# PaddlePaddle/PASSL

Measured on AMD Instinct MI355X. Metric: images/sec/node (2-view), MoCo-v2 R50 bs256/GPU, higher is better.
Workload: dtype bf16; 1 GPU; MoCo-v2 ResNet-50 bf16, bs=256/GPU, 2x224^2 synthetic views, queue=65536, dim=128, T=0.2, m=0.999, momentum-SGD (BASELINE configs[1]); global_batch=256, parallelism=dp1, allocator_retries=0

## Files before the change

include/passl_hip.h:

```cpp
#ifndef PASSL_HIP_H_
#define PASSL_HIP_H_

#include <stdint.h>

#ifdef __cplusplus
extern "C" {
#endif

typedef void* passl_stream_t;

enum passl_status {
  PASSL_OK = 0,
  PASSL_EINVAL = -1,
  PASSL_ELAUNCH = -2,
  PASSL_EUNSUPPORTED = -3
};

enum passl_dtype { PASSL_F32 = 0, PASSL_BF16 = 1 };

#define PASSL_HIP_ABI_VERSION 16
int passl_hip_abi_version(void);
int passl_hip_set_option(const char* name, int value);
int passl_hip_get_option(const char* name, int* value);
int passl_hip_last_igemm_kernel(void);
// ... 147 lines not shown
                           int C, int relu, int dtype, passl_stream_t stream);

int passl_hip_maxpool3x3s2_fwd(const void* x, void* y, uint8_t* idx, int N, int H, int W, int C,
                               int dtype, passl_stream_t stream);
int passl_hip_maxpool3x3s2_bwd(const void* dy, const uint8_t* idx, void* dx, int N, int H, int W,
                               int C, int dtype, passl_stream_t stream);
int passl_hip_bn_relu_maxpool_blocks(int N, int H, int W, int C);
int passl_hip_bn_relu_maxpool_fwd(const void* x, const float* scale, const float* shift, void* y, uint8_t* idx, int N,
                                  int H, int W, int C, int dtype, passl_stream_t stream);
int passl_hip_bn_relu_maxpool_bwd_reduce(const void* dy, const uint8_t* idx, const void* x, const float* mean,
                                         const float* invstd, const float* scale, const float* shift, float* partial,
                                         int nblocks, int N, int H, int W, int C, int dtype, passl_stream_t stream);
int passl_hip_bn_relu_maxpool_bwd_apply(const void* dy, const uint8_t* idx, const void* x, const float* coef,
                                        const float* scale, const float* shift, void* dx, int N, int H, int W, int C,
                                        int dtype, passl_stream_t stream);
int passl_hip_avgpool_fwd(const void* x, void* y, int N, int HW, int C, int dtype,
                          passl_stream_t stream);
int passl_hip_avgpool_bwd(const void* dy, void* dx, int N, int HW, int C, int dtype,
                          passl_stream_t stream);
int passl_hip_relu_bwd(const void* dy, const void* y, void* dx, int64_t n, int dtype,
                       passl_stream_t stream);
int passl_hip_colsum(const void* x, float* out, int64_t M, int C, int dtype, float* ws,
                     int64_t ws_floats, passl_stream_t stream);
int passl_hip_colsum_acc(const void* x, float* out, int64_t M, int C, int dtype, float* ws,
                         int64_t ws_floats, passl_stream_t stream);


int passl_hip_l2norm_fwd(const float* x, float* y, float* norm, int N, int D, float eps,
                         passl_stream_t stream);
int passl_hip_l2norm_bwd(const float* dy, const float* y, const float* norm, void* dx, int N,
// ... 197 lines not shown
```

passl_amd/csrc/bn_chunk.h:

```cpp
#pragma once
#include "common.h"

namespace bnc {

__device__ __forceinline__ void affine8(float (&v)[8], const float (&sc)[8], const float (&sh)[8]) {
#pragma unroll
  for (int e = 0; e < 8; ++e) v[e] = v[e] * sc[e] + sh[e];
}

__device__ __forceinline__ void relu8(float (&v)[8]) {
#pragma unroll
  for (int e = 0; e < 8; ++e) v[e] = fmaxf(v[e], 0.f);
}

__device__ __forceinline__ void bwd8(float (&o)[8], const float (&g)[8], const float (&v)[8], const float (&cA)[8],
                                     const float (&cB)[8], const float (&cC)[8]) {
#pragma unroll
  for (int e = 0; e < 8; ++e) o[e] = __fmaf_rn(cA[e], g[e], cB[e] * v[e]) + cC[e];
}

}
```

passl_amd/csrc/stem_pool.hip:

```cpp
#include "common.h"
#include "options.h"

namespace {

constexpr int kThreads = 256;
constexpr int kUnroll = 8;

template <typename T> __device__ __forceinline__ float round_to(float v);
template <> __device__ __forceinline__ float round_to<float>(float v) { return v; }
template <> __device__ __forceinline__ float round_to<bf16_t>(float v) { return bf2f(f2bf(v)); }

template <typename T>
__global__ void __launch_bounds__(kThreads) bn_relu_maxpool_fwd_kernel(const T* __restrict__ x,
                                                                       const float* __restrict__ scale,
                                                                       const float* __restrict__ shift,
                                                                       T* __restrict__ y, uint8_t* __restrict__ idx,
                                                                       int N, int H, int W, int C, int P, int Q) {
  const uint32_t cc = (uint32_t)C >> 3;
  const uint32_t total = (uint32_t)N * P * Q * cc;
  const uint32_t i = blockIdx.x * kThreads + threadIdx.x;
  if (i >= total) return;
  const int c8 = (int)(i % cc);
  uint32_t t = i / cc;
  const int q = (int)(t % (uint32_t)Q); t /= (uint32_t)Q;
// ... 236 lines not shown
template <typename T>
struct Item {
  uint32_t gw[2][2][kWords<T>];
  uint32_t ix[2][2][2];
  uint32_t xv[2][2][kWords<T>];
  uint32_t xb;
  uint32_t flags;
};

template <typename T>
__device__ __forceinline__ const T* at(const T* base, uint32_t elem_off) {
  return reinterpret_cast<const T*>(reinterpret_cast<const char*>(base) + (size_t)(elem_off * (uint32_t)sizeof(T)));
}

template <typename T>
__device__ __forceinline__ void load_item(Item<T>& it, const T* __restrict__ dy, const uint8_t* __restrict__ idx,
                                          const T* __restrict__ x, const Geo& g, uint32_t i, int c8) {
  const bool live = i < g.total;
  const uint32_t pix = (live ? i : g.total - 1) >> g.cshift;
  const uint32_t t1 = fdiv(pix, g.dW2);
  const uint32_t q2 = pix - t1 * g.W2;
  const uint32_t n = fdiv(t1, g.dH2);
  const uint32_t p2 = t1 - n * g.H2;
  const uint32_t C = (uint32_t)g.C;
  const bool pv = p2 + 1 < (uint32_t)g.P, qv = q2 + 1 < (uint32_t)g.Q;
  const bool hv = 2 * p2 + 1 < (uint32_t)g.H, wv = 2 * q2 + 1 < (uint32_t)g.W;
  const uint32_t ob = ((n * (uint32_t)g.P + p2) * (uint32_t)g.Q + q2) * C + (uint32_t)c8 * 8u;
  const uint32_t oa = pv ? (uint32_t)g.Q * C : 0u, oq = qv ? C : 0u;
  const uint32_t xb = ((n * (uint32_t)g.H + 2 * p2) * (uint32_t)g.W + 2 * q2) * C + (uint32_t)c8 * 8u;
  const uint32_t xa = hv ? (uint32_t)g.W * C : 0u, xq = wv ? C : 0u;
#pragma unroll
  for (int a = 0; a < 2; ++a)
#pragma unroll
    for (int b = 0; b < 2; ++b) {
      const uint32_t o = ob + (a ? oa : 0u) + (b ? oq : 0u);
      load_raw<T>(at<T>(dy, o), it.gw[a][b]);
      const uint2 t = *reinterpret_cast<const uint2*>(idx + (size_t)o);
      it.ix[a][b][0] = t.x; it.ix[a][b][1] = t.y;
    }
#pragma unroll
  for (int dh = 0; dh < 2; ++dh)
#pragma unroll
    for (int dw = 0; dw < 2; ++dw) load_raw<T>(at<T>(x, xb + (dh ? xa : 0u) + (dw ? xq : 0u)), it.xv[dh][dw]);
  it.xb = xb;
  const uint32_t l = live ? 1u : 0u, p1 = pv ? l : 0u, q1 = qv ? l : 0u, h1 = hv ? l : 0u, w1 = wv ? l : 0u;
  it.flags = l | (q1 << 1) | (p1 << 2) | ((p1 & q1) << 3) | (l << 4) | (w1 << 5) | (h1 << 6) | ((h1 & w1) << 7);
}

template <typename T>
__device__ __forceinline__ void pair_grad(const Item<T>& it, const uint32_t (&ix)[2][2][2], int k, const float (&sc)[2],
                                          const float (&sh)[2], float (&g)[2][2][2], float (&xf)[2][2][2]) {
  float w[2][2][2];
  uint32_t t[2][2][2];
#pragma unroll
  for (int a = 0; a < 2; ++a)
#pragma unroll
    for (int b = 0; b < 2; ++b)
#pragma unroll
      for (int j = 0; j < 2; ++j) {
        w[a][b][j] = elem<T>(it.gw[a][b], 2 * k + j);
        t[a][b][j] = __builtin_amdgcn_ubfe(ix[a][b][k >> 1], (uint32_t)(16 * (k & 1) + 8 * j), 8u);
// ... 104 lines not shown
#pragma unroll
  for (int e = 0; e < 8; ++e) { red[threadIdx.x * 16 + e] = a0[e]; red[threadIdx.x * 16 + 8 + e] = a1[e]; }
  __syncthreads();
  const uint32_t cc = 1u << g.cshift;
  if (threadIdx.x < cc) {
    float s0[8] = {0, 0, 0, 0, 0, 0, 0, 0}, s1[8] = {0, 0, 0, 0, 0, 0, 0, 0};
    for (uint32_t l = 0; l < kThreads / cc; ++l) {
      const uint32_t t = l * cc + threadIdx.x;
#pragma unroll
      for (int e = 0; e < 8; ++e) { s0[e] += red[t * 16 + e]; s1[e] += red[t * 16 + 8 + e]; }
    }
    float* o = partial + ((int64_t)blockIdx.x * g.C + threadIdx.x * 8) * 2;
#pragma unroll
    for (int e = 0; e < 8; e += 2) *reinterpret_cast<float4*>(o + e * 2) = make_float4(s0[e], s1[e], s0[e + 1], s1[e + 1]);
  }
}

}

bool shape_ok(int N, int H, int W, int C, int64_t* out_items, int64_t* in_items) {
  if (N <= 0 || H <= 0 || W <= 0 || C <= 0 || (C & 7) || (kThreads % (C >> 3)) != 0) return false;
  const int P = (H + 2 - 3) / 2 + 1, Q = (W + 2 - 3) / 2 + 1;
  *out_items = (int64_t)N * P * Q * (C >> 3);
  *in_items = (int64_t)N * ((H + 1) / 2) * ((W + 1) / 2) * (C >> 3);
  return *out_items <= 0x7fffffffll && *in_items <= 0x7fffffffll && (int64_t)N * H * W * C <= 0x7fffffff0ll;
}

v2::Geo make_geo(int N, int H, int W, int C, int64_t in_items) {
  v2::Geo g;
  g.H = H; g.W = W; g.C = C;
// ... 72 lines not shown
                                                   const float* scale, const float* shift, void* dx, int N, int H, int W,
                                                   int C, int dtype, passl_stream_t stream) {
  int64_t oi, ii;
  if (!dy || !idx || !x || !coef || !scale || !shift || !dx || !aligned16(dy) || !aligned16(x) || !aligned16(dx) ||
      !aligned16(coef) || !aligned16(scale) || !aligned16(shift) || (reinterpret_cast<uintptr_t>(idx) & 7))
    return PASSL_EINVAL;
  if (!shape_ok(N, H, W, C, &oi, &ii)) return PASSL_EUNSUPPORTED;
  const int P = (H + 2 - 3) / 2 + 1, Q = (W + 2 - 3) / 2 + 1;
  PASSL_DISPATCH_DTYPE(dtype, hipLaunchKernelGGL(bn_relu_maxpool_bwd_apply_kernel<T>, dim3((unsigned)((ii + kThreads - 1) / kThreads)),
                                                 dim3(kThreads), 0, as_stream(stream), reinterpret_cast<const T*>(dy), idx,
                                                 reinterpret_cast<const T*>(x), coef, scale, shift, reinterpret_cast<T*>(dx), N,
                                                 H, W, C, P, Q);)
  PASSL_RETURN_IF_LAUNCH_FAILED();
  return PASSL_OK;
}
```

passl_amd/hip/config.py:

```python
import os

import torch

_state = {'device': None, 'dtype': torch.bfloat16,
          'fused_bn_stats': os.environ.get('PASSL_FUSED_BN_STATS', '1') != '0',
          'fuse_residual_grad': os.environ.get('PASSL_FUSE_RESIDUAL_GRAD', '1') != '0',
          'fused_bn_backward': os.environ.get('PASSL_FUSED_BN_BACKWARD', '1') != '0',
          'fused_bn_backward2': os.environ.get('PASSL_FUSED_BN_BACKWARD2', '1') != '0',
          'overlap': os.environ.get('PASSL_OVERLAP', '1') != '0',
          'fork_downsample': os.environ.get('PASSL_FORK_DOWNSAMPLE', '1') != '0',
          'side_reductions': os.environ.get('PASSL_SIDE_REDUCTIONS', '1') != '0',
          'fused_stem_pool': os.environ.get('PASSL_FUSED_STEM_POOL', '1') != '0',
          'stem_wgrad_parts': max(1, int(os.environ.get('PASSL_STEM_WGRAD_PARTS', '2') or 1)),
          'stem_tail_flush': os.environ.get('PASSL_STEM_TAIL_FLUSH', '1') != '0',
          'stem_wgrad_main_last': os.environ.get('PASSL_STEM_WGRAD_MAIN_LAST', '1') != '0',
          'side_urgent_rows': int(os.environ.get('PASSL_SIDE_URGENT_ROWS', '500000') or 0),
          'wgrad_halo': int(os.environ.get('PASSL_WGRAD_HALO', '2') or 0),
          'igemm_a_bn': int(os.environ.get('PASSL_IGEMM_A_BN', '0') or 0) & 7,
          'igemm_a_bnb': int(os.environ.get('PASSL_IGEMM_A_BNB', '7') or 0) & 7}


def set_device(name):
    if isinstance(name, torch.device):
        _state['device'] = name
    elif name in ('gpu', 'cuda'):
        _state['device'] = torch.device('cuda', int(os.environ.get('PASSL_DEVICE_INDEX',
                                                                  os.environ.get('LOCAL_RANK', 0))))
        torch.cuda.set_device(_state['device'])
# ... 59 lines not shown
    return _state['fork_downsample']


def side_reductions():
    return _state['side_reductions']


def fused_stem_pool():
    return _state['fused_stem_pool']


def stem_wgrad_parts():
    return _state['stem_wgrad_parts']


def stem_wgrad_main_last():
    return _state['stem_wgrad_main_last']


def side_urgent_rows():
    return _state['side_urgent_rows']


def stem_tail_flush():
    return _state['stem_tail_flush']


def wgrad_halo():
    return _state['wgrad_halo']


def igemm_a_bn(channels):
    return bool(_state['igemm_a_bn'] & _ktile_bit(channels))


def igemm_a_bnb(channels):
    return bool(_state['igemm_a_bnb'] & _ktile_bit(channels))


def _ktile_bit(channels):
    nk = (channels + 63) // 64
    return 1 if nk == 1 else (2 if nk == 2 else 4)


_BOOL_FLAGS = ('fused_bn_stats', 'fuse_residual_grad', 'fused_bn_backward', 'overlap', 'fork_downsample',
               'side_reductions', 'fused_stem_pool', 'fused_bn_backward2', 'stem_tail_flush', 'stem_wgrad_main_last')
_INT_FLAGS = ('stem_wgrad_parts', 'side_urgent_rows', 'wgrad_halo', 'igemm_a_bn', 'igemm_a_bnb')


def set_flag(name, value):
    if name in _BOOL_FLAGS:
        _state[name] = bool(value)
    elif name in _INT_FLAGS:
        _state[name] = max(1, int(value)) if name == 'stem_wgrad_parts' else int(value)
        if name == 'wgrad_halo':
            from . import lib as L
            if L.loaded():
                L.check(L.load().passl_hip_set_option(b'wgrad_halo', int(value)), 'set_option wgrad_halo')
    else:
        raise KeyError('unknown flag %r (known: %s)' % (name, ', '.join(_BOOL_FLAGS + _INT_FLAGS)))

# ... 5 lines not shown
```

passl_amd/hip/lib.py:

```python
import ctypes as C
import os

import torch

_HERE = os.path.dirname(os.path.abspath(__file__))
LIB_PATH = os.path.join(os.path.dirname(_HERE), 'lib', 'libpassl_hip.so')

F32, BF16 = 0, 1
ABI_VERSION = 16
GRAD_CLIP_CHUNK = 16384
_DT = {torch.float32: F32, torch.bfloat16: BF16}

c_p = C.c_void_p
c_i = C.c_int
c_l = C.c_int64
c_f = C.c_float


class ConvDesc(C.Structure):
    _fields_ = [('a', c_p), ('b', c_p), ('y', c_p), ('scale', c_p), ('shift', c_p),
                ('residual', c_p), ('stats', c_p),
                ('bnb_y', c_p), ('bnb_mask', c_p), ('bnb_mean', c_p), ('bnb_invstd', c_p),
                ('bnb_scale', c_p), ('bnb_shift', c_p), ('bnb_partial', c_p),
                ('N', C.c_int32), ('OP', C.c_int32), ('OQ', C.c_int32), ('NCOLS', C.c_int32),
# ... 57 lines not shown
                                      c_i, c_p]),
    'passl_hip_bn_bwd_finalize': (c_i, [c_p, c_i, c_l, c_i, c_p, c_p, c_p, c_p, c_p, c_p, c_p]),
    'passl_hip_bn_moments': (c_i, [c_p, c_i, c_l, c_i, c_i, c_p, c_p]),
    'passl_hip_bn_finalize_moments': (c_i, [c_p, c_i, c_i, c_p, c_p, c_p, c_p, c_f, c_f, c_p, c_p, c_p, c_p, c_p]),
    'passl_hip_bn_bwd_sums': (c_i, [c_p, c_i, c_l, c_i, c_p, c_p]),
    'passl_hip_bn_bwd_finalize_sums': (c_i, [c_p, c_i, c_i, c_l, c_i, c_p, c_p, c_p, c_p, c_p, c_p, c_p]),
    'passl_hip_bn_bwd_apply': (c_i, [c_p, c_p, c_p, c_p, c_p, c_p, c_p, c_p, c_l, c_i, c_i, c_i,
                                     c_p]),
    'passl_hip_maxpool3x3s2_fwd': (c_i, [c_p, c_p, c_p, c_i, c_i, c_i, c_i, c_i, c_p]),
    'passl_hip_maxpool3x3s2_bwd': (c_i, [c_p, c_p, c_p, c_i, c_i, c_i, c_i, c_i, c_p]),
    'passl_hip_bn_relu_maxpool_blocks': (c_i, [c_i, c_i, c_i, c_i]),
    'passl_hip_bn_relu_maxpool_fwd': (c_i, [c_p, c_p, c_p, c_p, c_p, c_i, c_i, c_i, c_i, c_i, c_p]),
    'passl_hip_bn_relu_maxpool_bwd_reduce': (c_i, [c_p, c_p, c_p, c_p, c_p, c_p, c_p, c_p, c_i, c_i, c_i, c_i, c_i, c_i,
                                                   c_p]),
    'passl_hip_bn_relu_maxpool_bwd_apply': (c_i, [c_p, c_p, c_p, c_p, c_p, c_p, c_p, c_i, c_i, c_i, c_i, c_i, c_p]),
    'passl_hip_avgpool_fwd': (c_i, [c_p, c_p, c_i, c_i, c_i, c_i, c_p]),
    'passl_hip_avgpool_bwd': (c_i, [c_p, c_p, c_i, c_i, c_i, c_i, c_p]),
    'passl_hip_relu_bwd': (c_i, [c_p, c_p, c_p, c_l, c_i, c_p]),
    'passl_hip_colsum': (c_i, [c_p, c_p, c_l, c_i, c_i, c_p, c_l, c_p]),
    'passl_hip_colsum_acc': (c_i, [c_p, c_p, c_l, c_i, c_i, c_p, c_l, c_p]),
    'passl_hip_l2norm_fwd': (c_i, [c_p, c_p, c_p, c_i, c_i, c_f, c_p]),
    'passl_hip_l2norm_bwd': (c_i, [c_p, c_p, c_p, c_p, c_i, c_i, c_i, c_p]),
    'passl_hip_infonce_workspace_bytes': (c_l, [c_i, c_i]),
    'passl_hip_infonce_fwd': (c_i, [c_p, c_p, c_p, c_i, c_i, c_i, c_f, c_p, c_p, c_p, c_p, c_p]),
    'passl_hip_infonce_bwd_workspace_bytes': (c_l, [c_i, c_i]),
    'passl_hip_infonce_bwd': (c_i, [c_p, c_p, c_p, c_p, c_p, c_i, c_i, c_i, c_f, c_p, c_p, c_p]),
    'passl_hip_enqueue': (c_i, [c_p, c_p, c_i, c_i, c_i, c_i, c_p]),
    'passl_hip_enqueue_dev': (c_i, [c_p, c_p, c_i, c_i, c_p, c_i, c_p]),
    'passl_hip_lars_momentum': (c_i, [c_p, c_p, c_p, c_p, c_p, c_p, c_i, c_p, c_i, c_p, c_f, c_f,
                                      c_f, c_f, c_f, c_p]),
# ... 174 lines not shown
```

passl_amd/hip/nn.py:

```python
from types import SimpleNamespace

import torch
import torch.nn as tnn
from torch.autograd import Function

from . import config, ops, streams
from . import plan as P
from .packer import WeightPacker


class Layer(tnn.Module):

    def sublayers(self, include_self=False):
        mods = list(self.modules())
        return mods if include_self else mods[1:]

    def set_state_dict(self, sd, *a, **k):
        return self.load_state_dict(sd, *a, **k)


def _need_rt(layer):
    if getattr(layer, '_rt', None) is None:
        raise RuntimeError('%s is not attached to an EncoderArena (call EncoderArena(encoder) after '
                           'building the model)' % type(layer).__name__)
# ... 75 lines not shown


def dy_link(t):
    return getattr(t, '_passl_dy_link', None)


def _apply_in_consumer(conv, y, residual, relu, stats):
    g = conv.geom
    return (relu and residual is None and stats is not None and y.dtype == torch.bfloat16 and not conv.is_stem and
            g.k == 1 and g.stride == 1 and g.pad == 0 and g.cin == y.shape[-1] and g.cin % 64 == 0 and g.cin < 512 and
            g.cout > 64 and config.igemm_a_bn(g.cin))


class WgradLink:

    __slots__ = ('launch', 'done')

    def __init__(self):
        self.launch = None
        self.done = False


def wgrad_link(t):
    return getattr(t, '_passl_wgrad_link', None)


def _stem_wgrad(layer, pl, x, dy, tmp):
    ops.conv_wgrad(pl.wd, x, dy.reshape(-1, layer.geom.cout), tmp)


def _stem_wgrad_finish(layer, tmp):
    ops.unpad_add(tmp, layer._rt.dw, layer.geom.cout, 7, 7, 3, P.STEM_ROW // 4, 4)


# ... 10 lines not shown
        if pending is not None:
            done = ops.conv_igemm(pl.fd, pending.y, rt.w_fwd, y, stats=slab,
                                  apro=dict(mode=1, scale=pending.scale, shift=pending.shift, out=x))
            if done is None:
                ops.bn_apply(pending.y, pending.scale, pending.shift, None, True, out=x)
        if done is None:
            ops.conv_igemm(pl.fd, x, rt.w_fwd, y, stats=slab)
        if any(ctx.needs_input_grad):
            rt.arena.expect_grad(rt.indices)
        ctx.save_for_backward(x)
        ctx.layer, ctx.pl, ctx.hw = layer, pl, hw
        ctx.add_slot, ctx.sink_slot, ctx.producer = add_slot, sink_slot, producer
        ctx.side = streams.enabled(x)
        ctx.wlink = None
        ctx.dylink = dylink
        if wlink is not None and ctx.side and any(ctx.needs_input_grad):
            ctx.wlink = wlink
            state = {}

            def piece(dy_all, n0, n1, tmp):
                _stem_wgrad(layer, layer._plan(n1 - n0, hw[0], hw[1]), x[n0:n1], dy_all[n0:n1], tmp)

            def launch(dy_all, n0, n1, i, parts):
                dev = dy_all.device
                on_main = parts > 1 and config.stem_wgrad_main_last()
                if on_main and i == parts - 1:
                    tmp = ops.zeros(layer.geom.cout, P.STEM_K * P.STEM_ROW, dtype=torch.float32, device=dev)
                    piece(dy_all, n0, n1, tmp)
                    streams.wait_stream(torch.cuda.current_stream(dev), streams.side_stream(dev))
                    _stem_wgrad_finish(layer, tmp)
# ... 1 lines not shown
                with streams.on_side(dev, reads=(x, dy_all), in_backward=True):
                    if 'tmp' not in state:
                        state['tmp'] = ops.zeros(layer.geom.cout, P.STEM_K * P.STEM_ROW, dtype=torch.float32, device=dev)
                    piece(dy_all, n0, n1, state['tmp'])
                    if i == parts - (2 if on_main else 1):
                        _stem_wgrad_finish(layer, state.pop('tmp'))
            wlink.launch = launch
        return y

    @staticmethod
    def backward(ctx, dy):
        (x,) = ctx.saved_tensors
        layer, pl = ctx.layer, ctx.pl
        rt = layer._rt
        g = layer.geom
        streams.autograd_node_entry(dy.device)
        dy = dy.contiguous()
        dx = None
        late = ctx.dylink.take(dy) if ctx.dylink is not None else None
        if late is not None and not (ctx.needs_input_grad[0] and len(pl.dds) == 1 and not pl.dgrad_zero):
            ops.bn_bwd_apply_fused(late[0], late[1], late[2], dy)
            late = None
        if ctx.needs_input_grad[0]:
            N = x.shape[0]
            alloc = ops.zeros if pl.dgrad_zero else torch.empty
            dx = alloc(N, ctx.hw[0], ctx.hw[1], g.cin, dtype=dy.dtype, device=dy.device)
            extra = ctx.add_slot.take() if ctx.add_slot is not None else None
            if extra is not None and (len(pl.dds) != 1 or pl.dgrad_zero):
                raise RuntimeError('residual-gradient fusion needs a single dense data-gradient conv')
            link = ctx.producer
# ... 33 lines not shown
                    slab2 = None
            if fuse:
                link.fused = (slab, off)
                if slab2 is not None:
                    link.res_link.fused = (slab2, off)
            if ctx.sink_slot is not None:
                ctx.sink_slot.put(dx)
                dx = None
        def wgrad():
            if layer.is_stem:
                tmp = ops.zeros(g.cout, P.STEM_K * P.STEM_ROW, dtype=torch.float32, device=dy.device)
                _stem_wgrad(layer, pl, x, dy, tmp)
                _stem_wgrad_finish(layer, tmp)
            else:
                ops.conv_wgrad(pl.wd, x, dy.view(-1, g.cout), rt.dw)
        wl = ctx.wlink
        if wl is not None:
            wl.launch = None
        if wl is not None and wl.done:
            pass
        elif ctx.side:
            rows = config.side_urgent_rows()
            streams.side_later(dy.device, wgrad, reads=(x, dy), urgent=rows > 0 and dy.numel() // g.cout >= rows)
        else:
            wgrad()
        rt.arena.grad_ready(rt.indices)
        return dx, None, None, None, None, None, None, None, None, None, None


class Conv2D(Layer):

    def __init__(self, in_channels, out_channels, kernel_size, stride=1, padding=0, dilation=1,
                 groups=1, bias_attr=False, **_):
# ... 19 lines not shown
            else:
                dds, skipped = ([], False)
                if rt.dgrad_packs is not None:
                    dds, skipped = P.dgrad_plan(g, N, H, W, packs=rt.dgrad_packs)
                pl = SimpleNamespace(fd=P.fwd_desc(g, N, H, W), wd=P.wgrad_desc(g, N, H, W),
                                     dds=dds, dgrad_zero=skipped)
            self._plans[key] = pl
        return pl

    def forward(self, x, hw=None, want_stats=False, add_slot=None, sink_slot=None, producer=None, pending=None):
        if hw is None:
            hw = (x.shape[1], x.shape[2])
        stats = None
        if want_stats and x.dtype == torch.bfloat16 and config.fused_bn_stats():
            stats = ops.conv_stats_buffer(self._plan(x.shape[0], hw[0], hw[1]).fd, x.device)
        wlink = WgradLink() if (self.is_stem and config.stem_wgrad_parts() > 1) else None
        g = self.geom
        dylink = DyLink() if (torch.is_grad_enabled() and x.dtype == torch.bfloat16 and not self.is_stem and
                              g.k == 1 and g.stride == 1 and g.pad == 0 and g.cin <= 64 and g.cout % 64 == 0 and
                              g.cout < 512 and config.fused_bn_backward() and config.igemm_a_bnb(g.cout)) else None
        y = _ConvFn.apply(x, self.weight, self, hw, stats, add_slot, sink_slot, producer, wlink, pending, dylink)
        if dylink is not None:
            y._passl_dy_link = dylink
        if wlink is not None and wlink.launch is not None:
            y._passl_wgrad_link = wlink
        return (y, stats) if want_stats else y

    @torch.no_grad()
    def infer(self, x, bn=None, residual=None, relu=False, hw=None):
        rt = _need_rt(self)
        if hw is None:
            hw = (x.shape[1], x.shape[2])
        N = x.shape[0]
        pl = self._plan(N, hw[0], hw[1])
        y = torch.empty(N, pl.fd.OP, pl.fd.OQ, self.geom.cout, dtype=x.dtype, device=x.device)
        scale = shift = None
        if bn is not None:
            scale, shift = bn.infer_affine()
        ops.conv_igemm(pl.fd, x, rt.w_fwd, y, scale=scale, shift=shift, residual=residual, relu=relu)
# ... 167 lines not shown
            layer._rt.arena.expect_grad(layer._rt.indices)
        ctx.save_for_backward(y, st, idx)
        ctx.layer, ctx.wlink = layer, wlink
        return out

    @staticmethod
    def backward(ctx, dout):
        y, st, idx = ctx.saved_tensors
        layer, wl = ctx.layer, ctx.wlink
        streams.autograd_node_entry(dout.device)
        if config.stem_tail_flush():
            streams.flush_side(dout.device)
        for p in (layer.weight, layer.bias):
            if p.grad is None:
                p.grad = ops.zeros_like(p)
        piecewise = wl is not None and wl.launch is not None and not wl.done
        dx = ops.bn_relu_maxpool_bwd(dout.contiguous(), idx, y, layer.weight.detach(), st, layer.weight.grad,
                                     layer.bias.grad, parts=config.stem_wgrad_parts() if piecewise else 1,
                                     on_part=wl.launch if piecewise else None)
        if piecewise:
            wl.done = True
        if layer._rt is not None:
            layer._rt.arena.grad_ready(layer._rt.indices)
        return dx, None, None, None, None, None


def bn_relu_maxpool(bn, y, stats=None):
    fused = (config.fused_stem_pool() and torch.is_grad_enabled() and not bn.uses_global_stats() and bn.affine and
             not (getattr(bn, '_sync', False) and _collectives_active()) and y.is_cuda and
             ops.bn_relu_maxpool_supported(y))
    if not fused:
        return _MaxPoolFn.apply(bn(y, relu=True, stats=stats))
    return _BNReluMaxPoolFn.apply(y, bn.weight, bn.bias, bn, stats, wgrad_link(y))


# ... 608 lines not shown
```

passl_amd/hip/ops.py:

```python
import ctypes as C
import math

import torch

from . import config
from . import lib as L
from . import plan as P


def _lib():
    return L.load()


class _Workspace:

    def __init__(self):
        self._bufs = {}

    def get(self, n_floats, device):
        key = (device.type, device.index, L.stream() if device.type == 'cuda' else 0)
        buf = self._bufs.get(key)
        if buf is None or buf.numel() < n_floats:
            buf = torch.empty(max(int(n_floats), 1 << 20), dtype=torch.float32, device=device)
            self._bufs[key] = buf
# ... 349 lines not shown

def bn_relu_maxpool_supported(x):
    return x.dim() == 4 and _lib().passl_hip_bn_relu_maxpool_blocks(*x.shape) > 0


def bn_relu_maxpool_fwd(x, stats):
    N, H, W, Cc = x.shape
    P_, Q_ = (H + 2 - 3) // 2 + 1, (W + 2 - 3) // 2 + 1
    y = torch.empty(N, P_, Q_, Cc, dtype=x.dtype, device=x.device)
    idx = torch.empty(N, P_, Q_, Cc, dtype=torch.uint8, device=x.device)
    L.check(_lib().passl_hip_bn_relu_maxpool_fwd(L.ptr(x), L.ptr(stats[2]), L.ptr(stats[3]), L.ptr(y), L.ptr(idx),
                                                 N, H, W, Cc, L.dt(x), L.stream()), 'bn_relu_maxpool_fwd')
    return y, idx


def bn_relu_maxpool_bwd(dy, idx, x, gamma, stats, dgamma, dbeta, parts=1, on_part=None):
    N, H, W, Cc = x.shape
    lib, st, dtc, dev = _lib(), L.stream(), L.dt(x), x.device
    nb = lib.passl_hip_bn_relu_maxpool_blocks(N, H, W, Cc)
    partial = torch.empty(bn_partial_floats(nb, Cc, False), dtype=torch.float32, device=dev)
    coef = torch.empty(3 * Cc, dtype=torch.float32, device=dev)
    L.check(lib.passl_hip_bn_relu_maxpool_bwd_reduce(L.ptr(dy), L.ptr(idx), L.ptr(x), L.ptr(stats[0]), L.ptr(stats[1]),
                                                     L.ptr(stats[2]), L.ptr(stats[3]), L.ptr(partial), nb, N, H, W, Cc,
                                                     dtc, st), 'bn_relu_maxpool_bwd_reduce')
    L.check(lib.passl_hip_bn_bwd_finalize(L.ptr(partial), nb, N * H * W, Cc, L.ptr(gamma), L.ptr(stats[0]),
                                          L.ptr(stats[1]), L.ptr(dgamma), L.ptr(dbeta), L.ptr(coef), st),
            'bn_bwd_finalize')
    dx = torch.empty_like(x)
    parts = max(1, min(int(parts), N))
    for i in range(parts):
        n0, n1 = N * i // parts, N * (i + 1) // parts
        L.check(lib.passl_hip_bn_relu_maxpool_bwd_apply(L.ptr(dy[n0:n1]), L.ptr(idx[n0:n1]), L.ptr(x[n0:n1]), L.ptr(coef),
                                                        L.ptr(stats[2]), L.ptr(stats[3]), L.ptr(dx[n0:n1]), n1 - n0, H, W,
                                                        Cc, dtc, st), 'bn_relu_maxpool_bwd_apply')
        if on_part is not None:
            on_part(dx, n0, n1, i, parts)
    return dx


def avgpool_fwd(x):
    N, H, W, Cc = x.shape
    y = torch.empty(N, Cc, dtype=x.dtype, device=x.device)
# ... 788 lines not shown
```

Baseline: 11330 images/sec.

## Fuse stem BN-ReLU-maxpool backward with stem conv weight-gradient MFMA kernel

Adds a fused kernel that computes the stem BN/ReLU/maxpool input gradient on the fly in LDS and feeds it straight into a bf16 MFMA weight-gradient GEMM against the padded input, followed by a slab-reduction finish kernel. The stem's dx is never materialized and the separate conv wgrad pass is skipped, since the stem input needs no gradient. This removes a large write and re-read of the 112x112x64 activation gradient plus the separate apply and wgrad launches. In exchange it adds a per-WG fp32 workspace reduction, a rigid shape and layout (C=64, bf16, 4-channel padded input), and loses the overlap that the piecewise side-stream wgrad provided.

```diff
diff --git a/include/passl_hip.h b/include/passl_hip.h
--- a/include/passl_hip.h
+++ b/include/passl_hip.h
@@ -185,6 +185,11 @@
 int passl_hip_bn_relu_maxpool_bwd_apply(const void* dy, const uint8_t* idx, const void* x, const float* coef,
                                         const float* scale, const float* shift, void* dx, int N, int H, int W, int C,
                                         int dtype, passl_stream_t stream);
+int passl_hip_stem_wgrad_fused_blocks(int N, int H, int W, int C);
+int passl_hip_stem_wgrad_fused(const void* dout, const uint8_t* idx, const void* y, const float* coef, const float* scale,
+                               const float* shift, const void* xpad, float* ws, int nblocks, int N, int H, int W, int C,
+                               int Hp, int Wp, int dtype, passl_stream_t stream);
+int passl_hip_stem_wgrad_finish(const float* ws, int slabs, int parts, float* dw, int K, passl_stream_t stream);
 int passl_hip_avgpool_fwd(const void* x, void* y, int N, int HW, int C, int dtype,
                           passl_stream_t stream);
 int passl_hip_avgpool_bwd(const void* dy, void* dx, int N, int HW, int C, int dtype,
diff --git a/passl_amd/csrc/bn_chunk.h b/passl_amd/csrc/bn_chunk.h
--- a/passl_amd/csrc/bn_chunk.h
+++ b/passl_amd/csrc/bn_chunk.h
@@ -19,4 +19,8 @@
   for (int e = 0; e < 8; ++e) o[e] = __fmaf_rn(cA[e], g[e], cB[e] * v[e]) + cC[e];
 }
 
+__device__ __forceinline__ float bwd1(float g, float v, float cA, float cB, float cC) {
+  return __fmaf_rn(cA, g, cB * v) + cC;
 }
+
+}
diff --git a/passl_amd/csrc/stem_pool.hip b/passl_amd/csrc/stem_pool.hip
--- a/passl_amd/csrc/stem_pool.hip
+++ b/passl_amd/csrc/stem_pool.hip
@@ -1,3 +1,4 @@
+#include "bn_chunk.h"
 #include "common.h"
 #include "options.h"
 
@@ -274,6 +275,35 @@
 }
 
 template <typename T>
+__device__ __forceinline__ void load_item_at(Item<T>& it, const T* __restrict__ dy, const uint8_t* __restrict__ idx,
+                                             const T* __restrict__ x, const Geo& g, bool live, uint32_t n, uint32_t p2,
+                                             uint32_t q2, int c8) {
+  const uint32_t C = (uint32_t)g.C;
+  const bool pv = p2 + 1 < (uint32_t)g.P, qv = q2 + 1 < (uint32_t)g.Q;
+  const bool hv = 2 * p2 + 1 < (uint32_t)g.H, wv = 2 * q2 + 1 < (uint32_t)g.W;
+  const uint32_t ob = ((n * (uint32_t)g.P + p2) * (uint32_t)g.Q + q2) * C + (uint32_t)c8 * 8u;
+  const uint32_t oa = pv ? (uint32_t)g.Q * C : 0u, oq = qv ? C : 0u;
+  const uint32_t xb = ((n * (uint32_t)g.H + 2 * p2) * (uint32_t)g.W + 2 * q2) * C + (uint32_t)c8 * 8u;
+  const uint32_t xa = hv ? (uint32_t)g.W * C : 0u, xq = wv ? C : 0u;
+#pragma unroll
+  for (int a = 0; a < 2; ++a)
+#pragma unroll
+    for (int b = 0; b < 2; ++b) {
+      const uint32_t o = ob + (a ? oa : 0u) + (b ? oq : 0u);
+      load_raw<T>(at<T>(dy, o), it.gw[a][b]);
+      const uint2 t = *reinterpret_cast<const uint2*>(idx + (size_t)o);
+      it.ix[a][b][0] = t.x; it.ix[a][b][1] = t.y;
+    }
+#pragma unroll
+  for (int dh = 0; dh < 2; ++dh)
+#pragma unroll
+    for (int dw = 0; dw < 2; ++dw) load_raw<T>(at<T>(x, xb + (dh ? xa : 0u) + (dw ? xq : 0u)), it.xv[dh][dw]);
+  it.xb = xb;
+  const uint32_t l = live ? 1u : 0u, p1 = pv ? l : 0u, q1 = qv ? l : 0u, h1 = hv ? l : 0u, w1 = wv ? l : 0u;
+  it.flags = l | (q1 << 1) | (p1 << 2) | ((p1 & q1) << 3) | (l << 4) | (w1 << 5) | (h1 << 6) | ((h1 & w1) << 7);
+}
+
+template <typename T>
 __device__ __forceinline__ void load_item(Item<T>& it, const T* __restrict__ dy, const uint8_t* __restrict__ idx,
                                           const T* __restrict__ x, const Geo& g, uint32_t i, int c8) {
   const bool live = i < g.total;
@@ -282,29 +312,7 @@
   const uint32_t q2 = pix - t1 * g.W2;
   const uint32_t n = fdiv(t1, g.dH2);
   const uint32_t p2 = t1 - n * g.H2;
-  const uint32_t C = (uint32_t)g.C;
-  const bool pv = p2 + 1 < (uint32_t)g.P, qv = q2 + 1 < (uint32_t)g.Q;
-  const bool hv = 2 * p2 + 1 < (uint32_t)g.H, wv = 2 * q2 + 1 < (uint32_t)g.W;
-  const uint32_t ob = ((n * (uint32_t)g.P + p2) * (uint32_t)g.Q + q2) * C + (uint32_t)c8 * 8u;
-  const uint32_t oa = pv ? (uint32_t)g.Q * C : 0u, oq = qv ? C : 0u;
-  const uint32_t xb = ((n * (uint32_t)g.H + 2 * p2) * (uint32_t)g.W + 2 * q2) * C + (uint32_t)c8 * 8u;
-  const uint32_t xa = hv ? (uint32_t)g.W * C : 0u, xq = wv ? C : 0u;
-#pragma unroll
-  for (int a = 0; a < 2; ++a)
-#pragma unroll
-    for (int b = 0; b < 2; ++b) {
-      const uint32_t o = ob + (a ? oa : 0u) + (b ? oq : 0u);
-      load_raw<T>(at<T>(dy, o), it.gw[a][b]);
-      const uint2 t = *reinterpret_cast<const uint2*>(idx + (size_t)o);
-      it.ix[a][b][0] = t.x; it.ix[a][b][1] = t.y;
-    }
-#pragma unroll
-  for (int dh = 0; dh < 2; ++dh)
-#pragma unroll
-    for (int dw = 0; dw < 2; ++dw) load_raw<T>(at<T>(x, xb + (dh ? xa : 0u) + (dw ? xq : 0u)), it.xv[dh][dw]);
-  it.xb = xb;
-  const uint32_t l = live ? 1u : 0u, p1 = pv ? l : 0u, q1 = qv ? l : 0u, h1 = hv ? l : 0u, w1 = wv ? l : 0u;
-  it.flags = l | (q1 << 1) | (p1 << 2) | ((p1 & q1) << 3) | (l << 4) | (w1 << 5) | (h1 << 6) | ((h1 & w1) << 7);
+  load_item_at<T>(it, dy, idx, x, g, live, n, p2, q2, c8);
 }
 
 template <typename T>
@@ -439,6 +447,205 @@
 #pragma unroll
     for (int e = 0; e < 8; e += 2) *reinterpret_cast<float4*>(o + e * 2) = make_float4(s0[e], s1[e], s0[e + 1], s1[e + 1]);
   }
+}
+
+}
+
+namespace sw {
+
+typedef __attribute__((ext_vector_type(8))) __bf16 bf16x8_t;
+typedef __attribute__((ext_vector_type(4))) short s16x4;
+typedef __attribute__((ext_vector_type(8))) short s16x8;
+
+constexpr int kWgThreads = 512;
+constexpr int kMaxW = 128;
+constexpr int kK = 64, kJ = 224;
+constexpr int kXR = 9;
+constexpr int kXLoads = (kXR * (kMaxW + 3) + kWgThreads - 1) / kWgThreads;
+constexpr int kTabBytes = (kK / 2) * 3 * 16;
+constexpr int kTargetWgs = 256;
+constexpr int kFinishLanes = 16;
+
+struct Params {
+  const bf16_t* dout; const uint8_t* idx; const bf16_t* y; const bf16_t* xpad;
+  const float* coef; const float* scale; const float* shift;
+  float* ws;
+  v2::Geo g;
+  int N, Hp, Wp;
+  int groups;
+  int per_image, tiles_per_wg;
+  int xchunks, xpitch;
+  int dy_bytes, stage_bytes;
+};
+
+__device__ __forceinline__ int hswz8(int row) { return ((row >> 1) & 1) | (((row >> 3) & 1) << 1); }
+
+__device__ __forceinline__ s16x8 read_frag(const char* lo, const char* hi) {
+  const s16x4 a = __builtin_amdgcn_ds_read_tr16_b64_v4i16((__attribute__((address_space(3))) s16x4*)(lo));
+  const s16x4 b = __builtin_amdgcn_ds_read_tr16_b64_v4i16((__attribute__((address_space(3))) s16x4*)(hi));
+  return s16x8{a.x, a.y, a.z, a.w, b.x, b.y, b.z, b.w};
+}
+
+__global__ void __launch_bounds__(kWgThreads) stem_wgrad_fused_kernel(const Params p) {
+  extern __shared__ __attribute__((aligned(16))) char smem[];
+  float4* tab = reinterpret_cast<float4*>(smem + 2 * p.stage_bytes);
+  const int tid = threadIdx.x, lane = tid & 63, wave = tid >> 6;
+  if (tid < kK / 2) {
+    const int c = 2 * tid;
+    tab[tid * 3] = make_float4(p.scale[c], p.scale[c + 1], p.shift[c], p.shift[c + 1]);
+    tab[tid * 3 + 1] = make_float4(p.coef[c], p.coef[c + 1], p.coef[kK + c], p.coef[kK + c + 1]);
+    tab[tid * 3 + 2] = make_float4(p.coef[2 * kK + c], p.coef[2 * kK + c + 1], 0.f, 0.f);
+  }
+  const int W = p.g.W, rows = 2 * W;
+  for (int i = rows * 8 + tid; i < p.groups * 32 * 8; i += kWgThreads)
+#pragma unroll
+    for (int s = 0; s < 2; ++s) *reinterpret_cast<uint4*>(smem + s * p.stage_bytes + i * 16) = make_uint4(0u, 0u, 0u, 0u);
+  __syncthreads();
+  const int wm = wave >> 1, wn = wave & 1;
+  const int l15 = lane & 15, l4 = lane >> 4, r4 = (lane >> 2) & 3, c4 = lane & 3;
+
+  const int c8 = tid & 7;
+  const uint32_t q2 = (uint32_t)(tid >> 3);
+  const bool mine = q2 < p.g.W2;
+  uint32_t wr[2][2];
+  bool wr_ok[2][2];
+#pragma unroll
+  for (int dh = 0; dh < 2; ++dh)
+#pragma unroll
+    for (int dw = 0; dw < 2; ++dw) {
+      const int w = 2 * (int)q2 + dw, m = dh * W + w;
+      wr_ok[dh][dw] = mine && w < W;
+      wr[dh][dw] = (uint32_t)(m * (kK * 2) + ((((c8 >> 1) ^ hswz8(m)) << 5) | ((c8 & 1) << 4)));
+    }
+  uint32_t a_rd[2];
+#pragma unroll
+  for (int h = 0; h < 2; ++h) {
+    const int row = 8 * l4 + 4 * h + r4;
+    a_rd[h] = (uint32_t)(row * (kK * 2) + ((wm ^ hswz8(row)) << 5) + c4 * 8);
+  }
+
+  const int n = blockIdx.x / p.per_image;
+  const int t_begin = (blockIdx.x - n * p.per_image) * p.tiles_per_wg;
+  int tiles = t_begin + p.tiles_per_wg;
+  if (tiles > (int)p.g.H2) tiles = (int)p.g.H2;
+  v2::Item<bf16_t> it;
+  uint4 xr[kXLoads];
+  auto load_tile = [&](int t) {
+    v2::load_item_at<bf16_t>(it, p.dout, p.idx, p.y, p.g, mine, (uint32_t)n, (uint32_t)t, mine ? q2 : 0u, c8);
+#pragma unroll
+    for (int u = 0; u < kXLoads; ++u) {
+      const int e = tid + u * kWgThreads;
+      const int row = e / p.xchunks, ch = e - row * p.xchunks;
+      const int gr = 4 * t + row, gc = 2 * ch;
+      xr[u] = make_uint4(0u, 0u, 0u, 0u);
+      if (row < kXR && gr < p.Hp && gc < p.Wp)
+        xr[u] = *reinterpret_cast<const uint4*>(p.xpad + ((size_t)((uint32_t)(n * p.Hp + gr) * (uint32_t)p.Wp + (uint32_t)gc) << 2));
+    }
+  };
+
+  f32x4 acc[7];
+#pragma unroll
+  for (int j = 0; j < 7; ++j) acc[j] = f32x4{0.f, 0.f, 0.f, 0.f};
+
+  load_tile(t_begin);
+  for (int t = t_begin; t < tiles; ++t) {
+    char* sdy = smem + (t & 1) * p.stage_bytes;
+    char* sx = sdy + p.dy_bytes;
+    uint32_t w[2][2][4];
+    {
+      uint32_t ix[2][2][2];
+      v2::masked_idx<bf16_t>(it, ix);
+#pragma unroll
+      for (int k = 0; k < 4; ++k) {
+        const float4 t0 = tab[(c8 * 4 + k) * 3], t1 = tab[(c8 * 4 + k) * 3 + 1], t2 = tab[(c8 * 4 + k) * 3 + 2];
+        const float sc[2] = {t0.x, t0.y}, sh[2] = {t0.z, t0.w};
+        float gr[2][2][2], xf[2][2][2];
+        v2::pair_grad<bf16_t>(it, ix, k, sc, sh, gr, xf);
+#pragma unroll
+        for (int dh = 0; dh < 2; ++dh)
+#pragma unroll
+          for (int dw = 0; dw < 2; ++dw) {
+            const uint32_t pk = pack2bf(bnc::bwd1(gr[dh][dw][0], xf[dh][dw][0], t1.x, t1.z, t2.x),
+                                        bnc::bwd1(gr[dh][dw][1], xf[dh][dw][1], t1.y, t1.w, t2.y));
+            w[dh][dw][k] = ((it.flags >> (4 + dh * 2 + dw)) & 1u) ? pk : 0u;
+          }
+      }
+    }
+#pragma unroll
+    for (int dh = 0; dh < 2; ++dh)
+#pragma unroll
+      for (int dw = 0; dw < 2; ++dw)
+        if (wr_ok[dh][dw])
+          *reinterpret_cast<uint4*>(sdy + wr[dh][dw]) = make_uint4(w[dh][dw][0], w[dh][dw][1], w[dh][dw][2], w[dh][dw][3]);
+#pragma unroll
+    for (int u = 0; u < kXLoads; ++u) {
+      const int e = tid + u * kWgThreads;
+      const int row = e / p.xchunks, ch = e - row * p.xchunks;
+      if (row < kXR) *reinterpret_cast<uint4*>(sx + row * p.xpitch + ch * 16) = xr[u];
+    }
+    __syncthreads();
+    if (t + 1 < tiles) load_tile(t + 1);
+    for (int g = 0; g < p.groups; ++g) {
+      const s16x8 af = read_frag(sdy + g * 32 * (kK * 2) + a_rd[0], sdy + g * 32 * (kK * 2) + a_rd[1]);
+      uint32_t b_rd[2];
+#pragma unroll
+      for (int h = 0; h < 2; ++h) {
+        int m = 32 * g + 8 * l4 + 4 * h + r4;
+        m = m < rows ? m : 0;
+        const int hl = m >= W ? 1 : 0, wl = m - hl * W;
+        b_rd[h] = (uint32_t)(2 * hl * p.xpitch + (2 * wl + c4) * 8);
+      }
+      s16x8 bf[7];
+#pragma unroll
+      for (int j = 0; j < 7; ++j) {
+        const int jb = wn * 7 + j;
+        const int off = (jb >> 1) * p.xpitch + (jb & 1) * 32;
+        bf[j] = read_frag(sx + off + b_rd[0], sx + off + b_rd[1]);
+      }
+#pragma unroll
+      for (int j = 0; j < 7; ++j)
+        acc[j] = __builtin_amdgcn_mfma_f32_16x16x32_bf16(__builtin_bit_cast(bf16x8_t, af), __builtin_bit_cast(bf16x8_t, bf[j]),
+                                                         acc[j], 0, 0, 0);
+    }
+  }
+
+  float* o = p.ws + (size_t)blockIdx.x * (kK * kJ);
+#pragma unroll
+  for (int j = 0; j < 7; ++j)
+#pragma unroll
+    for (int r = 0; r < 4; ++r) o[(wm * 16 + l4 * 4 + r) * kJ + wn * 112 + j * 16 + l15] = acc[j][r];
+}
+
+__global__ void __launch_bounds__(kThreads) stem_wgrad_finish_kernel(const float* __restrict__ ws, int slabs, int parts,
+                                                                      float* __restrict__ dw, int K) {
+  constexpr int COLS = kThreads / kFinishLanes;
+  __shared__ float red[kFinishLanes][COLS];
+  const int col = threadIdx.x % COLS, zl = threadIdx.x / COLS;
+  const int o = blockIdx.x * COLS + col;
+  const bool live = o < K * 147;
+  const float* src = ws;
+  if (live) {
+    const int k = o / 147, rem = o - k * 147;
+    const int r = rem / 21, sc = rem - r * 21;
+    const int s = sc / 3, c = sc - s * 3;
+    src = ws + k * kJ + r * 32 + s * 4 + c;
+  }
+  float out = live && zl == 0 ? dw[o] : 0.f;
+  for (int i = 0; i < parts; ++i) {
+    const int z0 = (int)((int64_t)slabs * i / parts), z1 = (int)((int64_t)slabs * (i + 1) / parts);
+    const int cnt = z1 - z0, L = cnt <= 4 ? 1 : (cnt <= 32 ? 4 : 16);
+    float a = 0.f;
+    if (live && zl < L)
+      for (int z = z0 + zl; z < z1; z += L) a += src[(size_t)z * K * kJ];
+    __syncthreads();
+    red[zl][col] = a;
+    __syncthreads();
+    if (zl == 0 && cnt > 0) {
+      for (int l = 1; l < L; ++l) a += red[l][col];
+      out += a;
+    }
+  }
+  if (live && zl == 0) dw[o] = out;
 }
 
 }
@@ -541,3 +748,69 @@
   PASSL_RETURN_IF_LAUNCH_FAILED();
   return PASSL_OK;
 }
+
+namespace {
+
+bool stem_wgrad_geometry(int N, int H, int W, int C, sw::Params* p) {
+  int64_t oi, ii;
+  if (C != sw::kK || W > sw::kMaxW || !shape_ok(N, H, W, C, &oi, &ii) || (int64_t)N * H * W * C >= (1ll << 30)) return false;
+  p->g = make_geo(N, H, W, C, ii);
+  p->groups = (2 * W + 31) / 32;
+  p->xchunks = W + 3;
+  p->xpitch = (W + 4) * 16;
+  p->dy_bytes = p->groups * 32 * sw::kK * 2;
+  p->stage_bytes = p->dy_bytes + sw::kXR * p->xpitch;
+  const int H2 = (H + 1) / 2;
+  int want = sw::kTargetWgs / N;
+  want = want < 1 ? 1 : (want > H2 ? H2 : want);
+  p->tiles_per_wg = (H2 + want - 1) / want;
+  p->per_image = (H2 + p->tiles_per_wg - 1) / p->tiles_per_wg;
+  return true;
+}
+
+}
+
+extern "C" int passl_hip_stem_wgrad_fused_blocks(int N, int H, int W, int C) {
+  sw::Params p;
+  return stem_wgrad_geometry(N, H, W, C, &p) ? N * p.per_image : PASSL_EUNSUPPORTED;
+}
+
+extern "C" int passl_hip_stem_wgrad_fused(const void* dout, const uint8_t* idx, const void* y, const float* coef,
+                                          const float* scale, const float* shift, const void* xpad, float* ws,
+                                          int nblocks, int N, int H, int W, int C, int Hp, int Wp, int dtype,
+                                          passl_stream_t stream) {
+  if (!dout || !idx || !y || !coef || !scale || !shift || !xpad || !ws || !aligned16(dout) || !aligned16(y) ||
+      !aligned16(coef) || !aligned16(scale) || !aligned16(shift) || !aligned16(xpad) || !aligned16(ws) ||
+      (reinterpret_cast<uintptr_t>(idx) & 7))
+    return PASSL_EINVAL;
+  if (dtype != PASSL_BF16) return PASSL_EUNSUPPORTED;
+  sw::Params p;
+  if (!stem_wgrad_geometry(N, H, W, C, &p)) return PASSL_EUNSUPPORTED;
+  if (Hp < 2 * (H - 1) + 7 || Wp < 2 * (W - 1) + 8 || (Wp & 1) || (int64_t)N * Hp * Wp * 4 > 0x7fffffffll) return PASSL_EINVAL;
+  if ((int64_t)N * p.per_image > 0x7fffffffll || nblocks != N * p.per_image) return PASSL_EINVAL;
+  p.dout = reinterpret_cast<const bf16_t*>(dout); p.idx = idx; p.y = reinterpret_cast<const bf16_t*>(y);
+  p.xpad = reinterpret_cast<const bf16_t*>(xpad);
+  p.coef = coef; p.scale = scale; p.shift = shift; p.ws = ws;
+  p.N = N; p.Hp = Hp; p.Wp = Wp;
+  const int lds = 2 * p.stage_bytes + sw::kTabBytes;
+  static bool attr_set = false;
+  if (!attr_set) {
+    constexpr int max_lds = 2 * ((2 * sw::kMaxW + 31) / 32 * 32 * sw::kK * 2 + sw::kXR * (sw::kMaxW + 4) * 16) + sw::kTabBytes;
+    (void)hipFuncSetAttribute(reinterpret_cast<const void*>(&sw::stem_wgrad_fused_kernel),
+                              hipFuncAttributeMaxDynamicSharedMemorySize, max_lds);
+    attr_set = true;
+  }
+  hipLaunchKernelGGL(sw::stem_wgrad_fused_kernel, dim3((unsigned)nblocks), dim3(sw::kWgThreads), lds, as_stream(stream), p);
+  PASSL_RETURN_IF_LAUNCH_FAILED();
+  return PASSL_OK;
+}
+
+extern "C" int passl_hip_stem_wgrad_finish(const float* ws, int slabs, int parts, float* dw, int K, passl_stream_t stream) {
+  if (!ws || !dw || slabs <= 0 || parts <= 0 || K <= 0 || K > 4096 || !aligned16(ws) || (reinterpret_cast<uintptr_t>(dw) & 3))
+    return PASSL_EINVAL;
+  constexpr int cols = kThreads / sw::kFinishLanes;
+  hipLaunchKernelGGL(sw::stem_wgrad_finish_kernel, dim3((unsigned)((K * 147 + cols - 1) / cols)), dim3(kThreads), 0,
+                     as_stream(stream), ws, slabs, parts, dw, K);
+  PASSL_RETURN_IF_LAUNCH_FAILED();
+  return PASSL_OK;
+}
diff --git a/passl_amd/hip/config.py b/passl_amd/hip/config.py
--- a/passl_amd/hip/config.py
+++ b/passl_amd/hip/config.py
@@ -12,6 +12,7 @@
           'side_reductions': os.environ.get('PASSL_SIDE_REDUCTIONS', '1') != '0',
           'fused_stem_pool': os.environ.get('PASSL_FUSED_STEM_POOL', '1') != '0',
           'stem_wgrad_parts': max(1, int(os.environ.get('PASSL_STEM_WGRAD_PARTS', '2') or 1)),
+          'stem_wgrad_fused': os.environ.get('PASSL_STEM_WGRAD_FUSED', '1') != '0',
           'stem_tail_flush': os.environ.get('PASSL_STEM_TAIL_FLUSH', '1') != '0',
           'stem_wgrad_main_last': os.environ.get('PASSL_STEM_WGRAD_MAIN_LAST', '1') != '0',
           'side_urgent_rows': int(os.environ.get('PASSL_SIDE_URGENT_ROWS', '500000') or 0),
@@ -101,6 +102,10 @@
     return _state['stem_wgrad_parts']
 
 
+def stem_wgrad_fused():
+    return _state['stem_wgrad_fused']
+
+
 def stem_wgrad_main_last():
     return _state['stem_wgrad_main_last']
 
@@ -131,7 +136,8 @@
 
 
 _BOOL_FLAGS = ('fused_bn_stats', 'fuse_residual_grad', 'fused_bn_backward', 'overlap', 'fork_downsample',
-               'side_reductions', 'fused_stem_pool', 'fused_bn_backward2', 'stem_tail_flush', 'stem_wgrad_main_last')
+               'side_reductions', 'fused_stem_pool', 'fused_bn_backward2', 'stem_tail_flush', 'stem_wgrad_main_last',
+               'stem_wgrad_fused')
 _INT_FLAGS = ('stem_wgrad_parts', 'side_urgent_rows', 'wgrad_halo', 'igemm_a_bn', 'igemm_a_bnb')
 
 
diff --git a/passl_amd/hip/lib.py b/passl_amd/hip/lib.py
--- a/passl_amd/hip/lib.py
+++ b/passl_amd/hip/lib.py
@@ -95,6 +95,9 @@
     'passl_hip_bn_relu_maxpool_bwd_reduce': (c_i, [c_p, c_p, c_p, c_p, c_p, c_p, c_p, c_p, c_i, c_i, c_i, c_i, c_i, c_i,
                                                    c_p]),
     'passl_hip_bn_relu_maxpool_bwd_apply': (c_i, [c_p, c_p, c_p, c_p, c_p, c_p, c_p, c_i, c_i, c_i, c_i, c_i, c_p]),
+    'passl_hip_stem_wgrad_fused_blocks': (c_i, [c_i, c_i, c_i, c_i]),
+    'passl_hip_stem_wgrad_fused': (c_i, [c_p, c_p, c_p, c_p, c_p, c_p, c_p, c_p, c_i, c_i, c_i, c_i, c_i, c_i, c_i, c_i, c_p]),
+    'passl_hip_stem_wgrad_finish': (c_i, [c_p, c_i, c_i, c_p, c_i, c_p]),
     'passl_hip_avgpool_fwd': (c_i, [c_p, c_p, c_i, c_i, c_i, c_i, c_p]),
     'passl_hip_avgpool_bwd': (c_i, [c_p, c_p, c_i, c_i, c_i, c_i, c_p]),
     'passl_hip_relu_bwd': (c_i, [c_p, c_p, c_p, c_l, c_i, c_p]),
diff --git a/passl_amd/hip/nn.py b/passl_amd/hip/nn.py
--- a/passl_amd/hip/nn.py
+++ b/passl_amd/hip/nn.py
@@ -113,10 +113,11 @@
 
 class WgradLink:
 
-    __slots__ = ('launch', 'done')
+    __slots__ = ('launch', 'fused', 'done')
 
     def __init__(self):
         self.launch = None
+        self.fused = None
         self.done = False
 
 
@@ -157,6 +158,11 @@
         ctx.side = streams.enabled(x)
         ctx.wlink = None
         ctx.dylink = dylink
+        if (wlink is not None and config.stem_wgrad_fused() and x.dtype == torch.bfloat16 and
+                ctx.needs_input_grad[1] and not ctx.needs_input_grad[0]):
+            ctx.wlink = wlink
+            ctx.set_materialize_grads(False)
+            wlink.fused = lambda: (x, layer._rt.dw)
         if wlink is not None and ctx.side and any(ctx.needs_input_grad):
             ctx.wlink = wlink
             state = {}
@@ -188,6 +194,13 @@
         layer, pl = ctx.layer, ctx.pl
         rt = layer._rt
         g = layer.geom
+        wl = ctx.wlink
+        if dy is None:
+            if wl is None or not wl.done:
+                raise RuntimeError('convolution backward without an output gradient')
+            wl.launch = wl.fused = None
+            rt.arena.grad_ready(rt.indices)
+            return (None,) * 11
         streams.autograd_node_entry(dy.device)
         dy = dy.contiguous()
         dx = None
@@ -251,9 +264,8 @@
                 _stem_wgrad_finish(layer, tmp)
             else:
                 ops.conv_wgrad(pl.wd, x, dy.view(-1, g.cout), rt.dw)
-        wl = ctx.wlink
         if wl is not None:
-            wl.launch = None
+            wl.launch = wl.fused = None
         if wl is not None and wl.done:
             pass
         elif ctx.side:
@@ -303,7 +315,7 @@
         stats = None
         if want_stats and x.dtype == torch.bfloat16 and config.fused_bn_stats():
             stats = ops.conv_stats_buffer(self._plan(x.shape[0], hw[0], hw[1]).fd, x.device)
-        wlink = WgradLink() if (self.is_stem and config.stem_wgrad_parts() > 1) else None
+        wlink = WgradLink() if (self.is_stem and (config.stem_wgrad_parts() > 1 or config.stem_wgrad_fused())) else None
         g = self.geom
         dylink = DyLink() if (torch.is_grad_enabled() and x.dtype == torch.bfloat16 and not self.is_stem and
                               g.k == 1 and g.stride == 1 and g.pad == 0 and g.cin <= 64 and g.cout % 64 == 0 and
@@ -311,7 +323,7 @@
         y = _ConvFn.apply(x, self.weight, self, hw, stats, add_slot, sink_slot, producer, wlink, pending, dylink)
         if dylink is not None:
             y._passl_dy_link = dylink
-        if wlink is not None and wlink.launch is not None:
+        if wlink is not None and (wlink.launch is not None or wlink.fused is not None):
             y._passl_wgrad_link = wlink
         return (y, stats) if want_stats else y
 
@@ -509,11 +521,14 @@
         for p in (layer.weight, layer.bias):
             if p.grad is None:
                 p.grad = ops.zeros_like(p)
-        piecewise = wl is not None and wl.launch is not None and not wl.done
+        fused = (wl is not None and wl.fused is not None and not wl.done and config.stem_wgrad_fused() and
+                 ops.stem_wgrad_fused_supported(y))
+        piecewise = not fused and wl is not None and wl.launch is not None and not wl.done
         dx = ops.bn_relu_maxpool_bwd(dout.contiguous(), idx, y, layer.weight.detach(), st, layer.weight.grad,
-                                     layer.bias.grad, parts=config.stem_wgrad_parts() if piecewise else 1,
-                                     on_part=wl.launch if piecewise else None)
-        if piecewise:
+                                     layer.bias.grad, parts=config.stem_wgrad_parts() if piecewise or fused else 1,
+                                     on_part=wl.launch if piecewise else None,
+                                     fused_wgrad=wl.fused() if fused else None)
+        if piecewise or fused:
             wl.done = True
         if layer._rt is not None:
             layer._rt.arena.grad_ready(layer._rt.indices)
diff --git a/passl_amd/hip/ops.py b/passl_amd/hip/ops.py
--- a/passl_amd/hip/ops.py
+++ b/passl_amd/hip/ops.py
@@ -387,7 +387,11 @@
     return y, idx
 
 
-def bn_relu_maxpool_bwd(dy, idx, x, gamma, stats, dgamma, dbeta, parts=1, on_part=None):
+def stem_wgrad_fused_supported(x):
+    return x.dim() == 4 and x.dtype == torch.bfloat16 and _lib().passl_hip_stem_wgrad_fused_blocks(*x.shape) > 0
+
+
+def bn_relu_maxpool_bwd(dy, idx, x, gamma, stats, dgamma, dbeta, parts=1, on_part=None, fused_wgrad=None):
     N, H, W, Cc = x.shape
     lib, st, dtc, dev = _lib(), L.stream(), L.dt(x), x.device
     nb = lib.passl_hip_bn_relu_maxpool_blocks(N, H, W, Cc)
@@ -399,6 +403,18 @@
     L.check(lib.passl_hip_bn_bwd_finalize(L.ptr(partial), nb, N * H * W, Cc, L.ptr(gamma), L.ptr(stats[0]),
                                           L.ptr(stats[1]), L.ptr(dgamma), L.ptr(dbeta), L.ptr(coef), st),
             'bn_bwd_finalize')
+    if fused_wgrad is not None:
+        xpad, dw = fused_wgrad
+        slabs = lib.passl_hip_stem_wgrad_fused_blocks(N, H, W, Cc)
+        if slabs <= 0 or xpad.dim() != 4 or xpad.shape[0] != N or xpad.shape[3] != 4 or not xpad.is_contiguous():
+            raise L.PasslHipError('stem_wgrad_fused: unsupported shape %s over %s' % (tuple(x.shape), tuple(xpad.shape)))
+        ws = torch.empty(slabs * Cc * 224, dtype=torch.float32, device=dev)
+        L.check(lib.passl_hip_stem_wgrad_fused(L.ptr(dy), L.ptr(idx), L.ptr(x), L.ptr(coef), L.ptr(stats[2]), L.ptr(stats[3]),
+                                               L.ptr(xpad), L.ptr(ws), slabs, N, H, W, Cc, xpad.shape[1],
+                                               xpad.shape[2], dtc, st), 'stem_wgrad_fused')
+        L.check(lib.passl_hip_stem_wgrad_finish(L.ptr(ws), slabs, max(1, min(int(parts), N)), L.ptr(dw), Cc, st),
+                'stem_wgrad_finish')
+        return None
     dx = torch.empty_like(x)
     parts = max(1, min(int(parts), N))
     for i in range(parts):
```

After: 11440 images/sec (median of 6 runs). Within noise of the previous version (+1.0%).
